# lesterphillip/SVCC23_FastSVC

Hardware: AMD Instinct MI355X
Metric: audio samples/sec (24 kHz) FastSVC generator fwd (higher is better)
Workload: dtype bf16 (bf16 MFMA products, f32 accumulate; bf16 storage); 1 GPU; cfg3: 64 x 10 s utterances per GPU, F=1500 frames, T=240000 samples, generator fastsvc.yaml (144->[192,96,48,24], x[2,4,4,5]), spk_emb on; global_batch=64, utterance_samples=240000, parallelism=utterance-parallel x1

## Files before the change

svcc23_fastsvc_amd/csrc/fastsvc_hx.hip:

```cpp
#include "fastsvc_kernels.h"

namespace fastsvc {
#ifdef FASTSVC_ACT_2B
namespace FASTSVC_ACT_NS {
#endif

#include "fastsvc_device.inc"

#include "fastsvc_hx_common.inc"

template <int MW, int NW, bool RELOAD, bool OPT_LAST = false, int NS = 3 * MW * HX_NP, int SOFF = 0, bool ADV = true>
__device__ __forceinline__ void hx_unit_direct(f32x4 (&acc)[NW][MW], const unsigned char* tile, const int (&aoff)[3],
                                               int lo_off, HxWeightStream<NS>& ws, bool do_last = true) {
    constexpr int NSTEP = 3 * NW;
    constexpr int PF = HX_NP == 1 ? (MW >= 3 ? 2 : 3) : 1;
    HxFrag a[PF + 1];
    #pragma unroll
    for (int q = 0; q < PF && q < NSTEP; ++q) a[q] = hx_read(tile, aoff[q / NW] + (q % NW) * 16 * HX_ROW, lo_off);
    #pragma unroll
    for (int s = 0; s < NSTEP; ++s) {
        const int tap = s / NW, n = s % NW;
        if (s + PF < NSTEP) {
            a[(s + PF) % (PF + 1)] = hx_read(tile, aoff[(s + PF) / NW] + ((s + PF) % NW) * 16 * HX_ROW, lo_off);
            __builtin_amdgcn_sched_barrier(0);
        }
        if (!OPT_LAST || n + 1 < NW || do_last) hx_step<MW, OPT_LAST>(acc[n], a[s % (PF + 1)], &ws.wr[SOFF + tap * MW * HX_NP]);
        if (RELOAD && n + 1 == NW) {
            #pragma unroll
            for (int q = 0; q < MW * HX_NP; ++q) ws.request(SOFF + tap * MW * HX_NP + q);
        }
        __builtin_amdgcn_sched_barrier(0);
    }
    if (RELOAD && ADV) ws.advance();
}

template <int MW, int NW>
__device__ __forceinline__ void hx_unit_direct_wl(f32x4 (&acc)[NW][MW], const unsigned char* tile, const int (&aoff)[3],
                                                  int lo_off, const unsigned char* wl, int lane) {
    constexpr int NSTEP = 3 * NW;
    HxFrag a[2];
    u32x4 w[2][MW * HX_NP];
    a[0] = hx_read(tile, aoff[0], lo_off);
    #pragma unroll
    for (int q = 0; q < MW * HX_NP; ++q) w[0][q] = *reinterpret_cast<const u32x4*>(wl + q * HX_FRAG + lane * 16);
    #pragma unroll
    for (int s = 0; s < NSTEP; ++s) {
        const int tap = s / NW, n = s % NW;
        if (s + 1 < NSTEP) {
            a[(s + 1) & 1] = hx_read(tile, aoff[(s + 1) / NW] + ((s + 1) % NW) * 16 * HX_ROW, lo_off);
            if (n + 1 == NW) {
                #pragma unroll
                for (int q = 0; q < MW * HX_NP; ++q)
                    w[(tap + 1) & 1][q] = *reinterpret_cast<const u32x4*>(wl + ((tap + 1) * MW * HX_NP + q) * HX_FRAG + lane * 16);
            }
            __builtin_amdgcn_sched_barrier(0);
        }
        hx_step<MW>(acc[n], a[s & 1], &w[tap & 1][0]);
        __builtin_amdgcn_sched_barrier(0);
    }
}

template <int MW, int NW, bool RELOAD>
__device__ __forceinline__ void hx_unit_poly(f32x4 (&acc)[3][NW][MW], const unsigned char* tile, const int (&aoff)[3],
                                             int lo_off, HxWeightStream<3 * MW * HX_NP>& ws) {
    constexpr int NSTEP = 3 * NW;
    HxFrag side[2], mid[2];
// ... 328 lines not shown
        } else {
            u32x2v a0, a1, b0, b1;
            a0.x = wa.x; a0.y = wa.y; a1.x = wa.z; a1.y = wa.w; b0.x = wb.x; b0.y = wb.y; b1.x = wb.z; b1.y = wb.w;
            __builtin_amdgcn_raw_buffer_store_b64(a0, R.y, nvs >= 4 ? off : OOB_OFF, 0, FASTSVC_ST_AUX);
            __builtin_amdgcn_raw_buffer_store_b64(a1, R.y, nvs >= 8 ? off + 8 : OOB_OFF, 0, FASTSVC_ST_AUX);
            __builtin_amdgcn_raw_buffer_store_b64(b0, R.y2, nvs >= 4 ? off : OOB_OFF, 0, FASTSVC_ST_AUX);
            __builtin_amdgcn_raw_buffer_store_b64(b1, R.y2, nvs >= 8 ? off + 8 : OOB_OFF, 0, FASTSVC_ST_AUX);
        }
    }
    __builtin_amdgcn_fence(__ATOMIC_RELEASE, "wavefront");
    __builtin_amdgcn_wave_barrier();
    __builtin_amdgcn_fence(__ATOMIC_ACQUIRE, "wavefront");
}
template <int MW, int NW, int MODE> constexpr bool hx_dec2_staged() { return MODE == MODE_DEC2 && hx_dec2_patch_bytes<MW, NW>() <= 16 * 1024; }
template <int MW, int NW, int MODE, int EPI, int S>
constexpr bool hx_poly_staged() { return MODE == MODE_POLY && (EPI == EPI_AFF || EPI == EPI_PLAIN) && hx_poly_patch_bytes<MW, NW, S>() <= 16 * 1024; }
template <int MW, int NW, int MODE> constexpr bool hx_pairs_epi() { return MODE == MODE_DIRECT && NW % 2 == 0; }
#else
template <int MW, int NW, int MODE> constexpr bool hx_pairs_epi() { return false; }
template <int MW, int NW, int MODE, int EPI, int S> constexpr bool hx_poly_staged() { return false; }
template <int MW, int NW, int S> constexpr int hx_poly_patch_bytes() { return 0; }
template <int MW, int NW, int MODE> constexpr bool hx_dec2_staged() { return false; }
template <int MW, int NW> constexpr int hx_dec2_patch_bytes() { return 0; }
#endif

template <int MW, int NW, int MODE, int EPI>
constexpr bool hx_estage() {
    return MODE == MODE_DIRECT && (EPI == EPI_AFF || EPI == EPI_RES) && (hx_pairs_epi<MW, NW, MODE>() ? MW * NW <= 12 : MW * NW <= 6);
}

template <int MW, int NW, int MODE, int EPI>
constexpr bool hx_est2() { return hx_estage<MW, NW, MODE, EPI>() && MW * NW <= 4; }

template <int MW, int NW, int MODE, int EPI, int S = 1>
constexpr int hx_min_waves() {
#ifdef FASTSVC_ACT_2B
    if (MODE == MODE_DIRECT && MW == 2 && NW == 2 && EPI == EPI_AFF && S > 1) return 4;
#endif

    return (MODE == MODE_DIRECT && MW == 2 && (EPI == EPI_PLAIN || EPI == EPI_RANK1 || EPI == EPI_RES)) ? 4 : 2;
}

template <int MW, int NW, bool PAIRS>
__device__ __forceinline__ void hx_last_reduce(const ConvParams& p, const f32x4 (&acc)[NW][MW], const float (&kw)[MW],
                                               float bias, int b, int tcol0, int lane) {
    const __amdgpu_buffer_rsrc_t yr = make_rsrc(p.last_y + (long)b * p.last_y_b, p.ldy);
    #pragma unroll
    for (int n = 0; n < NW; ++n) {
        f32x4 s = acc[n][0] * kw[0];
        #pragma unroll
        for (int m = 1; m < MW; ++m) s += acc[n][m] * kw[m];
        #pragma unroll
        for (int e = 0; e < 4; ++e) {
            float v = s[e];
            v += __builtin_bit_cast(float, __builtin_amdgcn_mov_dpp(__builtin_bit_cast(int, v), 0xB1, 0xF, 0xF, true));
            v += __builtin_bit_cast(float, __builtin_amdgcn_mov_dpp(__builtin_bit_cast(int, v), 0x4E, 0xF, 0xF, true));
            v += __builtin_bit_cast(float, __builtin_amdgcn_mov_dpp(__builtin_bit_cast(int, v), 0x141, 0xF, 0xF, true));
            v += __builtin_bit_cast(float, __builtin_amdgcn_mov_dpp(__builtin_bit_cast(int, v), 0x140, 0xF, 0xF, true));
            s[e] = v;
        }
        const int t = PAIRS ? tcol0 + (n >> 1) * 32 + (lane >> 4) * 8 + (n & 1) * 4 : tcol0 + n * 16 + (lane >> 4) * 4;
        buf_store4(yr, ((lane & 15) == 0 && t < p.T) ? t * 4 : OOB_OFF, s + bias);
    }
}

#ifndef FASTSVC_HX_W8
#define FASTSVC_HX_W8 1
#endif
constexpr bool hx_w8(int MODE, bool tailk, int S) {
    return FASTSVC_HX_W8 != 0 && HX_NP == 1 && !tailk && (MODE == MODE_DIRECT || MODE == MODE_POLY || (MODE == MODE_DEC2 && S == 2));
}

template <int MW, int NW, int WM, int WN, int MODE, int EPI, int S, bool WSTATIC, bool TAILK = false>
__global__ __launch_bounds__(512, (hx_min_waves<MW, NW, MODE, EPI, S>()))
void conv_hx_kernel(const ConvParams p0) {
    constexpr bool UPH = MODE == MODE_UPHEAD;
    constexpr bool POLY = MODE == MODE_POLY, DEC2 = MODE == MODE_DEC2, CHAIN = MODE == MODE_CHAIN || MODE == MODE_CHAIN1 || UPH;
    constexpr bool IN1 = MODE == MODE_CHAIN1;
    constexpr bool WLB = MODE == MODE_CHAIN && S == 2;
    constexpr bool XR = MODE == MODE_DIRECT && S > 1;
    constexpr int NT = 16 * NW * WN;
    constexpr int NTV = CHAIN ? NT + 16 : NT;
    constexpr int HB = CHAIN ? 4 : 0;
    constexpr int NPROD_T = 256;
    constexpr bool W8 = hx_w8(MODE, TAILK, S);
    constexpr int SPARE = W8 ? 8 : 4;
    constexpr int MAXW = NTV + (MODE == MODE_DIRECT ? (W8 ? 64 : 56) : (W8 ? 16 : 8));
    constexpr int ITEMS = (MAXW + NPROD_T - 1) / NPROD_T;
    constexpr int NWS = DEC2 ? 4 : 3;
    constexpr int NVAR = DEC2 ? 2 : 1;
    constexpr int NSLOT = NWS * MW * HX_NP;
    constexpr bool TRACKS = AMAX_TRACK && ((CHAIN && MODE != MODE_UPHEAD) || (MODE == MODE_DIRECT && (EPI == EPI_RES || EPI == EPI_RANK1)));
    extern __shared__ __attribute__((aligned(16))) unsigned char smem_raw[];

    const int tid = threadIdx.x;
    const int lane = tid & 63;
    const int wave = __builtin_amdgcn_readfirstlane(tid >> 6);
    const bool producer = wave >= 4;
    const int cw = wave & 3;
    const int wave_m = cw / WN;
    const int wave_n = cw - wave_m * WN;
    const int z = blockIdx.z;
    const int sig = z / p0.B;
    const int b = z - sig * p0.B;
    ConvParams p = p0;
    if (p0.lens) {
        const int frames = p0.lens[b];
        p.T = frames * p0.len_mul;
        p.x_T = frames * p0.xlen_mul;
    }
    const int mg = blockIdx.y * WM + wave_m;
    const bool active = !producer && mg < p.ngroups;
    const int halo = (MODE == MODE_DIRECT || CHAIN) ? p.dil : 1;
    const int halo_al = W8 ? ((halo + 7) & ~7) : ((halo + 3) & ~3);
    const int W = NTV + 2 * halo_al;
    const int nch = p.nch32;
    const int CINp = nch * HX_KC;
    const int flags = p.flags;
    const int ntx = (p.T + NT - 1) / NT;
    const int tile0 = blockIdx.x * p.tpw;
    const int ntiles = min(p.tpw, ntx - tile0);
    if (ntiles <= 0) return;
    const int nunits = ntiles * (XR ? 2 * nch : nch);
#ifdef FASTSVC_TIMELINE
    const int wg_lin = blockIdx.x + gridDim.x * (blockIdx.y + gridDim.y * blockIdx.z);
    unsigned long long* tlw = (p.tl && wg_lin < p.tl_wgs) ? p.tl + ((long)wg_lin * 8 + wave) * 64 : nullptr;
    int tli = 0;
    auto stamp = [&](int tag) {
        if (tlw && lane == 0 && tli < 62) { tlw[tli++] = ((unsigned long long)tag << 56) | (__builtin_readcyclecounter() & 0x00ffffffffffffffull); }
    };
    stamp(1);
    if (tlw && lane == 0) {
        tlw[62] = __builtin_amdgcn_s_getreg(4 | (0 << 6) | (31 << 11));
        tlw[63] = __builtin_amdgcn_s_getreg(20 | (0 << 6) | (31 << 11));
    }
#else
    auto stamp = [](int) {};
#endif

    if constexpr (hx_min_waves<MW, NW, MODE, EPI, S>() >= 4) {
        const int wg_id = blockIdx.x + gridDim.x * (blockIdx.y + gridDim.y * blockIdx.z);
        if ((wg_id >> 8) & 1) {
            for (int k = 0; k < p.stagger; ++k) __builtin_amdgcn_s_sleep(16);
        }
    }
    double* sstat = reinterpret_cast<double*>(smem_raw);
    float2* ncoef = reinterpret_cast<float2*>(smem_raw + sizeof(double) * 2 * 16 * MW * WM);
    unsigned char* tiles = reinterpret_cast<unsigned char*>(ncoef + CINp + 8);
    __shared__ unsigned s_amax, s_cnt;
    __shared__ float s_inv[HX_NP == 2 ? 2 * 16 * MW * WM : 4];
    __shared__ __attribute__((aligned(16))) float s_mid[CHAIN ? 2 * (16 * MW * WM + 32) : 4];
    float sx = 1.f;
    float sx2 = 1.f;
    float s_mid_scale = 1.f;
    const int ninv = 16 * MW * p.ngroups;
    const float* invtab = (HX_NP == 2 && p.whx_inv) ? p.whx_inv + (long)sig * p.whx_inv_sig : nullptr;
    auto operand_scales = [&]() {
#ifndef FASTSVC_EXP_NOSCALE
        if constexpr (HX_NP == 2) {
            if (p.amax_in) {
                auto bound_of = [&](int entry, int s) -> float {
                    float bd = amax_read(p.amax_in, entry);
                    #pragma unroll
                    for (int j = 0; j < 2; ++j)
                        if (p.bnd_path[j]) { const float* q = p.bnd_path[j] + (long)s * p.bnd_sig[j]; bd = bd * q[0] + q[1]; }
                    return bd;
                };
                float bound = bound_of(sig * p.amax_in_sig + b, sig);
                if (p.amax_in2 > 0) bound = fmaxf(bound, bound_of(p.amax_in2 + b, 1));
                if (flags & F_PRE_NORM) bound += sqrtf((float)p.x_T);
                if constexpr (CHAIN) {
                    if (invtab) {
                        const float* cst = invtab + (UPH ? 3 : 2) * ninv;
// ... 466 lines not shown
            #pragma unroll
            for (int c = 0; c < 8; ++c) { i1w[c][0] *= sx; i1w[c][1] *= sx; i1w[c][2] *= sx; i1b[c] *= sx; }
        }
        pcommit(0, pa, oka, tiles);
        stamp(3);
        __syncthreads();
        stamp(4);
        for (int u = 0; u < nunits; u += 2) {
            pload(u + 2, pa, oka);
            stamp(9);
            pcommit(u + 1, pb, okb, tiles + bufsz);
            stamp(5);
            ppass2(u);
            __syncthreads();
            if (CHAIN && (u % nch) == nch - 1) __syncthreads();
            stamp(6);
            pload(u + 3, pb, okb);
            stamp(9);
            pcommit(u + 2, pa, oka, tiles);
            stamp(5);
            ppass2(u + 1);
            __syncthreads();
            if (CHAIN && u + 1 < nunits && ((u + 1) % nch) == nch - 1) __syncthreads();
            stamp(6);
        }
        }
    } else {
        f32x4 acc[(POLY || DEC2 || UPH) ? 1 : NW][MW];
        f32x4 acc3[3][(POLY || UPH) ? NW : 1][MW];
        f32x4 acc2[2][DEC2 ? NW : 1][MW];
        constexpr bool XSPLIT = XR && HX_NP == 2;
        f32x4 accX[XSPLIT ? NW : 1][MW];
        float s1[MW], s2[MW];
        constexpr bool GSTAT = MODE == MODE_DIRECT && (MW * NW <= 6 || (MW == 3 && NW == 4));
        double g1[GSTAT ? MW : 1], g2[GSTAT ? MW : 1];
        #pragma unroll
        for (int m = 0; m < (GSTAT ? MW : 1); ++m) g1[m] = g2[m] = 0.0;
        HxWeightStream<NSLOT> wst;
        const int wunits = UPH ? nch + 2 * p.nch32b : CHAIN ? nch + p.nch32b : XR ? 2 * nch : nch;
        wst.init(reinterpret_cast<const unsigned char*>(p.whx) + (long)sig * p.whx_sig +
                     (long)(active ? mg : 0) * wunits * NSLOT * HX_FRAG, WLB ? nch : wunits, lane);
        int aoff[3];
        #pragma unroll
        for (int tap = 0; tap < 3; ++tap)
            aoff[tap] = hx_lds_off((halo_al - halo) + tap * halo + wave_n * (NW * 16) + (lane & 15), lane >> 4);
        int aoffX[3];
        #pragma unroll
        for (int tap = 0; tap < 3; ++tap)
            aoffX[tap] = XR ? hx_lds_off((halo_al - 1) + tap + wave_n * (NW * 16) + (lane & 15), lane >> 4) : 0;
        HxWeightStream<NSLOT> wstX_static;
        if constexpr (XR && WSTATIC)
            wstX_static.init(reinterpret_cast<const unsigned char*>(p.whx) + (long)sig * p.whx_sig +
                                 ((long)(active ? mg : 0) * wunits + 1) * NSLOT * HX_FRAG, 1, lane);
        HxWeightStream<NSLOT>& wstX = (XR && WSTATIC) ? wstX_static : wst;
        EpiRsrc R;
        {
            const long ct = (long)p.COUT * p.ldy;
            const float* nul = p.bias;
            R.y = act_rsrc(p.y ? p.y : nul, p.y ? (long)sig * p.y_sig + (long)b * p.y_b : 0, p.y ? ct : 0);
            const bool has_y2 = DEC2 || (flags & F_AFF_OUT) != 0;
            R.y2 = act_rsrc(has_y2 ? p.y2 : nul, has_y2 ? (long)sig * p.y2_sig + (long)b * p.y2_b : 0, has_y2 ? ct : 0);
            R.res = act_rsrc(p.res ? p.res : nul, p.res ? (long)sig * p.res_sig + (long)b * p.res_b : 0, p.res ? ct : 0);
            const bool has_ss = (flags & (F_STATS | F_AFF_OUT)) != 0;
            R.ss = act_rsrc(has_ss ? p.ss_out : nul, has_ss ? (long)b * p.ss_out_b : 0, has_ss ? 2 * ct : 0);
            R.r1x = make_rsrc(p.r1x ? p.r1x + (long)sig * p.r1x_sig + (long)b * p.r1x_b : nul, p.r1x ? p.ldy : 0);
        }
        float k_bias[MW], k_bias2[MW], k_r1w[MW], k_r1b[MW];
// ... 15 lines not shown
        float t_inv[MW], t_inv2[MW];
        #pragma unroll
        for (int m = 0; m < MW; ++m) {
            const int cot = (mg * MW + m) * 16 + (lane & 15);
            const bool cok = active && cot < p.COUT;
            t_inv[m] = cok ? 1.f : 0.f; t_inv2[m] = t_inv[m];
            if constexpr (HX_NP == 2) {
                if (invtab) {
                    t_inv[m] = cok ? invtab[(CHAIN ? ninv : 0) + cot] : 0.f;
                    if constexpr (DEC2) t_inv2[m] = cok ? invtab[ninv + cot] : 0.f;
                    if constexpr (UPH) t_inv2[m] = cok ? invtab[2 * ninv + cot] : 0.f;
                    if constexpr (XR) t_inv2[m] = cok ? invtab[ninv + cot] : 0.f;
                }
            }
        }
        constexpr bool LAST_OK = MODE == MODE_DIRECT && EPI == EPI_RES && WM == 1;
        float k_last[MW];
        const float b_last = (LAST_OK && p.last_w) ? __builtin_bit_cast(float, __builtin_amdgcn_readfirstlane(__builtin_bit_cast(int, p.last_b[0]))) : 0.f;
        #pragma unroll
        for (int m = 0; m < MW; ++m) {
            const int cot = (mg * MW + m) * 16 + (lane & 15);
            k_last[m] = (LAST_OK && p.last_w && active && cot < p.COUT) ? p.last_w[cot] : 0.f;
        }
        constexpr bool EST = hx_estage<MW, NW, MODE, EPI>();
        constexpr bool PAIRS = hx_pairs_epi<MW, NW, MODE>();
        constexpr int EST_WAVE_FLOATS = EST ? (PAIRS ? MW * (NW / 2) * 256 : MW * NW * EST_ITEM_FLOATS) : 0;
        const int est_ops = EPI == EPI_RES ? 1 : p.res ? 3 : 2;
        const float* Ew = reinterpret_cast<const float*>(tiles + 2 * bufsz) + cw * (est_ops * EST_WAVE_FLOATS);
        constexpr bool EST2 = hx_est2<MW, NW, MODE, EPI>() && WSTATIC && !XR;
        const int est_set = 4 * est_ops * EST_WAVE_FLOATS;
        float* Xw = const_cast<float*>(reinterpret_cast<const float*>(tiles + 2 * bufsz)) + (EST2 ? 2 : 1) * est_set +
                    cw * (16 * 36);
        (void)Xw;
        stamp(2);
        setup_shared();
        if constexpr (HX_NP == 2) {
            const float isx = 1.0f / (CHAIN ? s_mid_scale : sx);
            if (lane < 16) {
                #pragma unroll
                for (int m = 0; m < MW; ++m) {
                    const int li = (wave_m * MW + m) * 16 + lane;
                    s_inv[li] = t_inv[m] * isx;
                    if constexpr (DEC2 || UPH) s_inv[16 * MW * WM + li] = t_inv2[m] * isx;
                }
            }
        }
        float xratio[MW];
        #pragma unroll
        for (int m = 0; m < MW; ++m) {
            xratio[m] = 0.f;
            if constexpr (XR && HX_NP == 2) {
                auto ex = [](float v) { return (int)((__builtin_bit_cast(unsigned, v) >> 23) & 0xffu); };
                const int e = ex(t_inv2[m]) - ex(t_inv[m]) + ex(sx) - ex(sx2) + 127;
                if (t_inv[m] != 0.f) xratio[m] = __builtin_bit_cast(float, (unsigned)min(254, max(1, e)) << 23);
            }
        }
        __syncthreads();
        stamp(4);
        int u = 0;
        if constexpr (CHAIN) {
            f32x4 accA[NW + 1][MW];
            const int cmidp = p.nch32b * HX_KC;
            auto fwd = [&](int m) -> float {
                if constexpr (HX_NP == 2) return __builtin_bit_cast(float, (254u << 23) - __builtin_bit_cast(unsigned, K.inv(m)));
                else return 1.f;
            };
// ... 113 lines not shown
                for (int m = 0; m < MW; ++m) { s1[m] = 0.f; s2[m] = 0.f; }
                ws_epilogue_kind<MW, NW, EPI_PLAIN, false, 0, 1>(p, R, acc, s1, s2, sig, mg, tcol0, active, lane, K, Ew);
                if constexpr (TRACKS) { if (p.amax_out) amax_tile_flush(R); }
                stamp(8);
                }
            }
        } else if constexpr (XR) {
            for (int tl = 0; tl < ntiles; ++tl) {
                #pragma unroll
                for (int n = 0; n < NW; ++n)
                    #pragma unroll
                    for (int m = 0; m < MW; ++m) {
                        acc[n][m] = f32x4{0.f, 0.f, 0.f, 0.f};
                        if constexpr (XSPLIT) accX[n][m] = f32x4{0.f, 0.f, 0.f, 0.f};
                    }
                const int tcolw = (tile0 + tl) * NT + wave_n * (NW * 16);
                for (int ch = 0; ch < nch; ++ch) {
                    if constexpr (EST) {
                        if (active && ch + 1 == nch) {
#ifdef FASTSVC_ACT_2B
                            if constexpr (PAIRS) hx_epilogue8_stage<MW, NW / 2, EPI>(p, R, Ew, mg, tcolw, lane);
                            else
#endif
                            ws_epilogue_stage<MW, NW, EPI>(p, R, Ew, mg, tcolw, lane);
                        }
                    }
                    if (active) hx_unit_direct<MW, NW, !WSTATIC>(acc, tiles, aoff, lo_off, wst);
                    stamp(7);
                    __syncthreads();
                    stamp(6);
                    ++u;
                    if (active) {
                        if constexpr (XSPLIT) hx_unit_direct<MW, NW, !WSTATIC>(accX, tiles + bufsz, aoffX, lo_off, wstX);
                        else hx_unit_direct<MW, NW, !WSTATIC>(acc, tiles + bufsz, aoffX, lo_off, wstX);
                    }
                    stamp(7);
                    if (ch + 1 == nch) {
                        if constexpr (XSPLIT) {
                            #pragma unroll
                            for (int n = 0; n < NW; ++n)
                                #pragma unroll
                                for (int m = 0; m < MW; ++m) acc[n][m] += accX[n][m] * xratio[m];
                        }
                        #pragma unroll
                        for (int m = 0; m < MW; ++m) { s1[m] = 0.f; s2[m] = 0.f; }
                        if constexpr (EST) { if (active) ws_epilogue_stage_wait<NSLOT>(!WSTATIC); }
#ifdef FASTSVC_ACT_2B
                        if constexpr (PAIRS) hx_epilogue8<MW, NW / 2, EPI, EST, false, false>(p, R, acc, s1, s2, sig, mg, tcolw, active, lane, K, Ew, Xw);
                        else
#endif
                        ws_epilogue_kind<MW, NW, EPI, EST, 0, -1>(p, R, acc, s1, s2, sig, mg, tcolw, active, lane, K, Ew);
                        if (flags & F_STATS) {
                            #pragma unroll
                            for (int m = 0; m < MW; ++m) {
                                if constexpr (GSTAT) { g1[m] += (double)s1[m]; g2[m] += (double)s2[m]; }
                                else {
                                    float a1 = s1[m], a2 = s2[m];
                                    a1 = row_xsum(a1); a2 = row_xsum(a2);
                                    if (active && lane < 16) {
                                        const int slot = ((wave_m * MW + m) * 16 + lane) * 2;
                                        atomicAdd(&sstat[slot + 0], (double)a1);
                                        atomicAdd(&sstat[slot + 1], (double)a2);
                                    }
                                }
                            }
                        }
                    }
                    stamp(8);
                    __syncthreads();
                    stamp(6);
                    ++u;
                }
            }
        } else
        for (int tl = 0; tl < ntiles; ++tl) {
            auto est_stage = [&](const float* slots, int tile) {
                if constexpr (EST) {
#ifdef FASTSVC_ACT_2B
                    if constexpr (PAIRS) hx_epilogue8_stage<MW, NW / 2, EPI>(p, R, slots, mg, tile * NT + wave_n * (NW * 16), lane);
                    else
#endif
                    ws_epilogue_stage<MW, NW, EPI>(p, R, slots, mg, tile * NT + wave_n * (NW * 16), lane);
                }
            };
            #pragma unroll
            for (int n = 0; n < NW; ++n)
                #pragma unroll
                for (int m = 0; m < MW; ++m) {
                    if constexpr (POLY) { acc3[0][n][m] = acc3[1][n][m] = acc3[2][n][m] = f32x4{0.f, 0.f, 0.f, 0.f}; }
                    else if constexpr (DEC2) { acc2[0][n][m] = acc2[1][n][m] = f32x4{0.f, 0.f, 0.f, 0.f}; }
                    else acc[n][m] = f32x4{0.f, 0.f, 0.f, 0.f};
                }
            const float* EwT = EST2 ? Ew + (tl & 1) * est_set : Ew;
            for (int ch = 0; ch < nch; ++ch, ++u) {
                if constexpr (EST2) {
                    if (active && !(FASTSVC_DBG_ON(p, DBG_NO_EPILOGUE))) {
                        if (tl == 0) est_stage(Ew, tile0);
                        if (tl + 1 < ntiles) est_stage(Ew + ((tl + 1) & 1) * est_set, tile0 + tl + 1);
                    }
                } else if constexpr (EST) {
                    if (active && ch == max(nch - 2, 0) && !(FASTSVC_DBG_ON(p, DBG_NO_EPILOGUE))) est_stage(Ew, tile0 + tl);
                }
                if (active && !(FASTSVC_DBG_ON(p, DBG_NO_MFMA))) {
                    if constexpr (POLY) hx_unit_poly<MW, NW, !WSTATIC>(acc3, tiles + (u & 1) * bufsz, aoff, lo_off, wst);
                    else if constexpr (DEC2) hx_unit_dec2<MW, NW, !WSTATIC>(acc2, tiles + (u & 1) * bufsz, aoff, lo_off, raw_off, wst);
                    else hx_unit_direct<MW, NW, !WSTATIC>(acc, tiles + (u & 1) * bufsz, aoff, lo_off, wst);
                }
                stamp(7);
                if (ch + 1 == nch) {
                    #pragma unroll
                    for (int m = 0; m < MW; ++m) { s1[m] = 0.f; s2[m] = 0.f; }
                    if constexpr (EST2) {
                        if (active) {
                            constexpr int PER_OP = PAIRS ? MW * (NW / 2) : MW * NW * EST_DMA_PER_ITEM;
                            constexpr int EITEMS = PAIRS ? MW * (NW / 2) : MW * NW;
                            const int ndma = tl + 1 < ntiles ? (EPI == EPI_RES ? 1 : p.res ? 3 : 2) * PER_OP : 0;
                            int nst = 0;
                            if (tl > 0 && !(FASTSVC_DBG_ON(p, DBG_NO_EPILOGUE))) {
                                if (EPI == EPI_AFF) nst = EITEMS * (p.y ? 2 : 1);
                                else nst = (p.y ? EITEMS : 0) + ((LAST_OK && p.last_w) ? NW : 0);
                            }
                            hx_wait_vmcnt(ndma + nst);
                        }
                    } else
                    if constexpr (EST) { if (active) ws_epilogue_stage_wait<NSLOT>(!WSTATIC && !(FASTSVC_DBG_ON(p, DBG_NO_MFMA))); }
                    stamp(10);
                    if constexpr (POLY) {
#ifdef FASTSVC_ACT_2B
                        if constexpr (hx_poly_staged<MW, NW, MODE, EPI, S>()) {
                            const int tcolw = (tile0 + tl) * NT + wave_n * (NW * 16);
                            unsigned char* Pw = tiles + 2 * bufsz + cw * hx_poly_patch_bytes<MW, NW, S>();
                            HxPolyPass2<MW, NW, EPI, S, 0, hx_poly_mc<MW>()> P2;
                            if (active) {
                                P2.request(p, R, mg, tcolw, lane);
                                hx_poly_pass1<MW, NW, S>(p, acc3, mg, lane, K, Pw);
                            }
                            __syncthreads();
                            if (active) P2.run(p, R, Pw, s1, s2, mg, tcolw, lane);
                        } else
                            hx_epilogue_poly8<MW, NW, EPI, S, TAILK>(p, R, acc3, s1, s2, mg, (tile0 + tl) * NT + wave_n * (NW * 16), active, lane, K);
#else
                        ws_epilogue_poly<MW, NW, EPI, S, TAILK ? 2 : 0>(p, R, acc3, s1, s2, mg, (tile0 + tl) * NT + wave_n * (NW * 16), active, lane, K);
#endif
                    }
                    else if constexpr (DEC2)
                    {
#ifdef FASTSVC_ACT_2B
                        if constexpr (hx_dec2_staged<MW, NW, MODE>())
                            hx_epilogue_dec2_staged<MW, NW>(p, R, acc2, sig, mg, (tile0 + tl) * NT + wave_n * (NW * 16), active, lane, K,
                                                            tiles + 2 * bufsz + cw * hx_dec2_patch_bytes<MW, NW>());
                        else
#endif
                        ws_epilogue_dec2<MW, NW>(p, R, acc2, sig, mg, (tile0 + tl) * NT + wave_n * (NW * 16), active, lane, K);
                    }
                    else {
#ifdef FASTSVC_ACT_2B
                        if constexpr (PAIRS) {
                            if (!(FASTSVC_DBG_ON(p, DBG_NO_EPILOGUE)))
                                hx_epilogue8<MW, NW / 2, EPI, EST, TAILK>(p, R, acc, s1, s2, sig, mg,
                                                                   (tile0 + tl) * NT + wave_n * (NW * 16), active, lane, K, EwT, Xw);
                        } else
#endif
                        ws_epilogue_kind<MW, NW, EPI, EST, TAILK ? 2 : 0, -1>(p, R, acc, s1, s2, sig, mg,
                                                              (tile0 + tl) * NT + wave_n * (NW * 16), active, lane, K, EwT);
                        if constexpr (LAST_OK) {
                            if (p.last_w && !(FASTSVC_DBG_ON(p, DBG_NO_EPILOGUE)))
                                hx_last_reduce<MW, NW, PAIRS>(p, acc, k_last, b_last, b, (tile0 + tl) * NT + wave_n * (NW * 16), lane);
                        }
                    }
                    stamp(11);
                    if constexpr (TRACKS) { if (p.amax_out) amax_tile_flush(R); }
                    if ((flags & F_STATS) && !(FASTSVC_DBG_ON(p, DBG_NO_EPILOGUE))) {
                        #pragma unroll
                        for (int m = 0; m < MW; ++m) {
                            if constexpr (GSTAT) { g1[m] += (double)s1[m]; g2[m] += (double)s2[m]; }
                            else {
                                float a1 = s1[m], a2 = s2[m];
                                a1 = row_xsum(a1); a2 = row_xsum(a2);
                                if (active && lane < 16) {
                                    const int slot = ((wave_m * MW + m) * 16 + lane) * 2;
                                    atomicAdd(&sstat[slot + 0], (double)a1);
                                    atomicAdd(&sstat[slot + 1], (double)a2);
                                }
                            }
                        }
                    }
                }
                stamp(8);
                __syncthreads();
                stamp(6);
            }
        }
        if constexpr (TRACKS) amax_flush(p, R, &s_amax, &s_cnt, 4, sig, b, lane, blockIdx.x);
        if constexpr (GSTAT) {
            if ((flags & F_STATS) && !(FASTSVC_DBG_ON(p, DBG_NO_EPILOGUE))) {
                #pragma unroll
                for (int m = 0; m < MW; ++m) {
                    double a1 = g1[m], a2 = g2[m];
                    a1 += __shfl_xor(a1, 16); a2 += __shfl_xor(a2, 16);
                    a1 += __shfl_xor(a1, 32); a2 += __shfl_xor(a2, 32);
                    if (active && lane < 16) {
                        const int slot = ((wave_m * MW + m) * 16 + lane) * 2;
                        atomicAdd(&sstat[slot + 0], a1);
                        atomicAdd(&sstat[slot + 1], a2);
                    }
                }
            }
        }
        if (nunits & 1) __syncthreads();
    }
    if ((flags & F_STATS) && !(FASTSVC_DBG_ON(p, DBG_NO_EPILOGUE))) {
        __syncthreads();
        for (int i = tid; i < 2 * 16 * MW * WM; i += 512) {
            const int co = blockIdx.y * (WM * MW * 16) + (i >> 1);
            if (co < p.COUT) atomicAdd(&p.st_out[((long)b * p.COUT + co) * 2 + (i & 1)], sstat[i]);
        }
    }
}

constexpr size_t HX_STATIC_LDS = 4096;
template <auto KERNEL>
static hipError_t hx_launch_instance(dim3 grid, size_t smem, hipStream_t stream, const ConvParams& p) {
    if (smem + HX_STATIC_LDS > 64 * 1024) {
        static const hipError_t attr = hipFuncSetAttribute(reinterpret_cast<const void*>(KERNEL),
                                                           hipFuncAttributeMaxDynamicSharedMemorySize, 160 * 1024 - HX_STATIC_LDS);
        if (attr != hipSuccess) return attr;
    }
    hipLaunchKernelGGL(KERNEL, grid, dim3(512), smem, stream, p);
    return hipGetLastError();
}

// ... 45 lines not shown
    } else if constexpr (MODE == MODE_CHAIN) {
        if (aff || smem + HX_STATIC_LDS > 160 * 1024) return hipErrorInvalidValue;
        const int kind = p.r1x ? EPI_RANK1 : p.res ? EPI_RES : EPI_PLAIN;
        const size_t wl = (size_t)p.nch32b * 3 * MW * HX_NP * HX_FRAG;
        if constexpr (WM == 1 && MW == 3) {
            if (kind == EPI_PLAIN && p.ngroups == 1 && p.nch32b > 1 && smem + wl + HX_STATIC_LDS <= 160 * 1024)
                return hx_launch_kind<MW, NW, WM, WN, MODE_CHAIN, EPI_PLAIN, 2>(grid, smem + wl, stream, p);
        }
#define FASTSVC_HXC(k) if (kind == k) return hx_launch_kind<MW, NW, WM, WN, MODE_CHAIN, k, 1>(grid, smem, stream, p);
        FASTSVC_HXC(EPI_PLAIN) FASTSVC_HXC(EPI_RES) FASTSVC_HXC(EPI_RANK1)
#undef FASTSVC_HXC
        return hipErrorInvalidValue;
    } else if constexpr (MODE == MODE_DEC2) {
        const size_t patch = hx_dec2_staged<MW, NW, MODE_DEC2>() ? 4 * (size_t)hx_dec2_patch_bytes<MW, NW>() : 0;
        if (p.s == 1 && (p.ldx & 3) == 0) return hx_launch_kind<MW, NW, WM, WN, MODE_DEC2, EPI_PLAIN, 2>(grid, smem + patch, stream, p);
        return hx_launch_kind<MW, NW, WM, WN, MODE_DEC2, EPI_PLAIN, 1>(grid, smem + patch, stream, p);
    } else if constexpr (MODE == MODE_POLY) {
#define FASTSVC_HXP(sv) \
        if (p.s == sv) return aff ? hx_launch_kind<MW, NW, WM, WN, MODE_POLY, EPI_AFF, sv>(grid, smem + (hx_poly_staged<MW, NW, MODE_POLY, EPI_AFF, sv>() ? 4 * hx_poly_patch_bytes<MW, NW, sv>() : 0), stream, p) \
                                  : hx_launch_kind<MW, NW, WM, WN, MODE_POLY, EPI_PLAIN, sv>(grid, smem + (hx_poly_staged<MW, NW, MODE_POLY, EPI_PLAIN, sv>() ? 4 * hx_poly_patch_bytes<MW, NW, sv>() : 0), stream, p);
        FASTSVC_HXP(2) FASTSVC_HXP(4) FASTSVC_HXP(5)
#undef FASTSVC_HXP
        return hipErrorInvalidValue;
    } else {
        const int kind = aff ? EPI_AFF : p.r1x ? EPI_RANK1 : p.res ? EPI_RES : EPI_PLAIN;
        size_t est = 0;
        constexpr bool PAIRS = hx_pairs_epi<MW, NW, MODE_DIRECT>();
        if ((kind == EPI_AFF && hx_estage<MW, NW, MODE_DIRECT, EPI_AFF>()) || (kind == EPI_RES && hx_estage<MW, NW, MODE_DIRECT, EPI_RES>()))
            est = sizeof(float) * 4 * (size_t)(aff ? (p.res ? 3 : 2) : 1) * (PAIRS ? MW * (NW / 2) * 256 : MW * NW * EST_ITEM_FLOATS);
        if (MW == 2 && p.nch32 == 1 && !p.x2 &&
            ((kind == EPI_AFF && hx_est2<MW, NW, MODE_DIRECT, EPI_AFF>()) || (kind == EPI_RES && hx_est2<MW, NW, MODE_DIRECT, EPI_RES>())))
            est *= 2;
        if (PAIRS) est += sizeof(float) * 4 * 16 * 36;
        if (p.x2) {
            if (kind != EPI_AFF || p.res || p.x2_T * p.s2 != p.T || (p.lens && (((p.len_mul | p.xlen_mul) & 3) != 0)))
                return hipErrorInvalidValue;
            if (w8 && p.s2 == 2 && W / p.s2 + 5 > 128) return hipErrorInvalidValue;
            if (w8 && !conv_hx_x2_rows_ok(p)) return hipErrorInvalidValue;
#define FASTSVC_HXX(sv, stat) if (p.s2 == sv) return hx_launch_instance<&conv_hx_kernel<MW, NW, WM, WN, MODE_DIRECT, EPI_AFF, sv, stat>>(grid, smem + est, stream, p);
            if constexpr (MW * NW <= 12) {
                if constexpr (MW == 2) { if (p.nch32 == 1) { FASTSVC_HXX(5, true) } }
                else { FASTSVC_HXX(2, false) FASTSVC_HXX(4, false) }
            }
#undef FASTSVC_HXX
            return hipErrorInvalidValue;
        }
#define FASTSVC_HX(k) if (kind == k) return hx_launch_kind<MW, NW, WM, WN, MODE_DIRECT, k, 1>(grid, smem + est, stream, p);
        FASTSVC_HX(EPI_PLAIN) FASTSVC_HX(EPI_RES) FASTSVC_HX(EPI_RANK1) FASTSVC_HX(EPI_AFF)
#undef FASTSVC_HX
        return hipErrorInvalidValue;
    }
}

hipError_t launch_conv_hx(const ConvParams& p, const ConvLaunch& cfg, hipStream_t stream) {
    if (p.ntaps != 3 || (p.T & 3) || !p.whx || p.nch32 * HX_KC > 512) return hipErrorInvalidValue;
#define FASTSVC_HXS(md, mw, nw, wm, wn) \
    if (cfg.MW == mw && cfg.NW == nw && cfg.WM == wm && cfg.WN == wn) \
        return hx_launch_shape<mw, nw, wm, wn, md>(p, cfg.nsig, stream);
    if (p.mode == MODE_DIRECT) {
        if (p.dil < 1 || p.dil > 28) return hipErrorInvalidValue;
        FASTSVC_HXS(MODE_DIRECT, 2, 2, 1, 4) FASTSVC_HXS(MODE_DIRECT, 2, 3, 1, 4)
        FASTSVC_HXS(MODE_DIRECT, 3, 2, 1, 4) FASTSVC_HXS(MODE_DIRECT, 3, 3, 1, 4)
        FASTSVC_HXS(MODE_DIRECT, 3, 4, 2, 2) FASTSVC_HXS(MODE_DIRECT, 3, 6, 2, 2)
        FASTSVC_HXS(MODE_DIRECT, 3, 8, 4, 1)
    } else if (p.mode == MODE_POLY) {
        if (p.dil != 1) return hipErrorInvalidValue;
// ... 58 lines not shown
```

svcc23_fastsvc_amd/csrc/fastsvc_hx_common.inc:

```

#ifdef FASTSVC_ACT_2B
#ifdef FASTSVC_ACT_F16
typedef _Float16 hx_t;
#else
typedef __bf16 hx_t;
#endif
constexpr int HX_NP = 1;
#else
typedef _Float16 hx_t;
constexpr int HX_NP = 2;
#endif
typedef hx_t hx8 __attribute__((ext_vector_type(8)));
typedef hx_t hx2 __attribute__((ext_vector_type(2)));

__device__ __forceinline__ f32x4 hx_mfma(hx8 a, hx8 b, f32x4 c) {
#if defined(FASTSVC_ACT_2B) && !defined(FASTSVC_ACT_F16)
    return __builtin_amdgcn_mfma_f32_16x16x32_bf16(a, b, c, 0, 0, 0);
#else
    return __builtin_amdgcn_mfma_f32_16x16x32_f16(a, b, c, 0, 0, 0);
#endif
}

template <bool IN1> struct HxWin { typedef act4_t type; };
template <> struct HxWin<true> { typedef f32x4 type; };
// ... 5 lines not shown
    return ((row ^ ((row >> 2) & 1)) * HX_ROW) + ((oct ^ ((row >> 1) & 2)) << 4);
}

__device__ __forceinline__ void hx_wait_vmcnt(int n) {
    if (n >= 20) asm volatile("s_waitcnt vmcnt(20)" ::: "memory");
    else if (n >= 16) asm volatile("s_waitcnt vmcnt(16)" ::: "memory");
    else if (n >= 12) asm volatile("s_waitcnt vmcnt(12)" ::: "memory");
    else if (n >= 10) asm volatile("s_waitcnt vmcnt(10)" ::: "memory");
    else if (n >= 8) asm volatile("s_waitcnt vmcnt(8)" ::: "memory");
    else if (n >= 6) asm volatile("s_waitcnt vmcnt(6)" ::: "memory");
    else if (n >= 4) asm volatile("s_waitcnt vmcnt(4)" ::: "memory");
    else if (n >= 3) asm volatile("s_waitcnt vmcnt(3)" ::: "memory");
    else if (n >= 2) asm volatile("s_waitcnt vmcnt(2)" ::: "memory");
    else if (n >= 1) asm volatile("s_waitcnt vmcnt(1)" ::: "memory");
    else asm volatile("s_waitcnt vmcnt(0)" ::: "memory");
}

template <int NSLOT>
struct HxWeightStream {
    u32x4 wr[NSLOT];
    __amdgpu_buffer_rsrc_t rsrc;
    int voff, next, total;
    __device__ __forceinline__ void init(const unsigned char* group_base, int nunits, int lane) {
        total = nunits * NSLOT * HX_FRAG;
        rsrc = __builtin_amdgcn_make_buffer_rsrc(const_cast<unsigned char*>(group_base), 0, total, 0x00020000);
        voff = lane * 16;
        #pragma unroll
        for (int s = 0; s < NSLOT; ++s) wr[s] = __builtin_amdgcn_raw_buffer_load_b128(rsrc, voff, s * HX_FRAG, 0);
        next = NSLOT * HX_FRAG;
        if (next >= total) next = 0;
    }
    __device__ __forceinline__ void request(int s) { wr[s] = __builtin_amdgcn_raw_buffer_load_b128(rsrc, voff, next + s * HX_FRAG, 0); }
    __device__ __forceinline__ void advance() { next += NSLOT * HX_FRAG; if (next >= total) next = 0; }
};

struct HxFrag { hx8 p[HX_NP]; };

__device__ __forceinline__ HxFrag hx_read(const unsigned char* tile, int off, int lo_off) {
    HxFrag f;
    f.p[0] = *reinterpret_cast<const hx8*>(tile + off);
    if constexpr (HX_NP == 2) f.p[1] = *reinterpret_cast<const hx8*>(tile + lo_off + off);
    return f;
}

template <int PROD, bool SWAP = false>
__device__ __forceinline__ f32x4 hx_prod(const HxFrag& a, const u32x4 (&w)[HX_NP], f32x4 acc) {
    constexpr int ia = (HX_NP == 2 && PROD == 2) ? 1 : 0, iw = (HX_NP == 2 && PROD == 1) ? 1 : 0;
    if constexpr (SWAP) return hx_mfma(__builtin_bit_cast(hx8, w[iw]), a.p[ia], acc);
    else return hx_mfma(a.p[ia], __builtin_bit_cast(hx8, w[iw]), acc);
}
constexpr int HX_NPROD = HX_NP == 2 ? 3 : 1;

template <int MW, bool SWAP = false>
__device__ __forceinline__ void hx_step(f32x4 (&acc)[MW], const HxFrag& a, const u32x4* w ) {
    #pragma unroll
    for (int pr = 0; pr < HX_NPROD; ++pr)
        #pragma unroll
        for (int m = 0; m < MW; ++m) {
            u32x4 wm[HX_NP];
            #pragma unroll
            for (int q = 0; q < HX_NP; ++q) wm[q] = w[m * HX_NP + q];
            if (pr == 0) acc[m] = hx_prod<0, SWAP>(a, wm, acc[m]);
            else if (pr == 1) acc[m] = hx_prod<1, SWAP>(a, wm, acc[m]);
            else acc[m] = hx_prod<2, SWAP>(a, wm, acc[m]);
        }
}
// ... 207 lines not shown
```

Before: 1.769 billion samples/s.

## Raise occupancy for MW3xNW2 affine conv by spilling stats to LDS and deferring weight reload

For the bf16 direct-mode MW=3,NW=2 affine conv kernel, raises the launch-bounds minimum waves to 4 so more waves fit per SIMD. To cut register pressure, the double-precision stats accumulators move from registers into a per-wave LDS area. The weight-stream reload for the last channel chunk is held back and issued after the epilogue, so those registers are not live across it. The cost is extra LDS traffic and a weight-load latency that the epilogue may no longer hide, plus a possible spill risk if the register budget is still too tight.

```diff
diff --git a/svcc23_fastsvc_amd/csrc/fastsvc_hx.hip b/svcc23_fastsvc_amd/csrc/fastsvc_hx.hip
--- a/svcc23_fastsvc_amd/csrc/fastsvc_hx.hip
+++ b/svcc23_fastsvc_amd/csrc/fastsvc_hx.hip
@@ -9,9 +9,9 @@
 
 #include "fastsvc_hx_common.inc"
 
-template <int MW, int NW, bool RELOAD, bool OPT_LAST = false, int NS = 3 * MW * HX_NP, int SOFF = 0, bool ADV = true>
+template <int MW, int NW, bool RELOAD, bool OPT_LAST = false, int NS = 3 * MW * HX_NP, int SOFF = 0, bool ADV = true, bool HOLD = false>
 __device__ __forceinline__ void hx_unit_direct(f32x4 (&acc)[NW][MW], const unsigned char* tile, const int (&aoff)[3],
-                                               int lo_off, HxWeightStream<NS>& ws, bool do_last = true) {
+                                               int lo_off, HxWeightStream<NS>& ws, bool do_last = true, bool hold = false) {
     constexpr int NSTEP = 3 * NW;
     constexpr int PF = HX_NP == 1 ? (MW >= 3 ? 2 : 3) : 1;
     HxFrag a[PF + 1];
@@ -25,13 +25,13 @@
             __builtin_amdgcn_sched_barrier(0);
         }
         if (!OPT_LAST || n + 1 < NW || do_last) hx_step<MW, OPT_LAST>(acc[n], a[s % (PF + 1)], &ws.wr[SOFF + tap * MW * HX_NP]);
-        if (RELOAD && n + 1 == NW) {
+        if (RELOAD && n + 1 == NW && !(HOLD && hold)) {
             #pragma unroll
             for (int q = 0; q < MW * HX_NP; ++q) ws.request(SOFF + tap * MW * HX_NP + q);
         }
         __builtin_amdgcn_sched_barrier(0);
     }
-    if (RELOAD && ADV) ws.advance();
+    if (RELOAD && ADV && !(HOLD && hold)) ws.advance();
 }
 
 template <int MW, int NW>
@@ -426,8 +426,19 @@
 template <int MW, int NW, int MODE, int EPI>
 constexpr bool hx_est2() { return hx_estage<MW, NW, MODE, EPI>() && MW * NW <= 4; }
 
-template <int MW, int NW, int MODE, int EPI, int S = 1>
+template <int MW, int NW, int MODE, int EPI, bool TAILK = false>
+constexpr bool hx_two_cu() {
+#ifdef FASTSVC_ACT_2B
+    return MODE == MODE_DIRECT && MW == 3 && NW == 2 && EPI == EPI_AFF && !TAILK;
+#else
+    return false;
+#endif
+}
+template <int MW> constexpr int hx_gsum_bytes() { return 4 * MW * 2 * 64 * (int)sizeof(double); }
+
+template <int MW, int NW, int MODE, int EPI, int S = 1, bool TAILK = false>
 constexpr int hx_min_waves() {
+    if (hx_two_cu<MW, NW, MODE, EPI, TAILK>()) return 4;
 #ifdef FASTSVC_ACT_2B
     if (MODE == MODE_DIRECT && MW == 2 && NW == 2 && EPI == EPI_AFF && S > 1) return 4;
 #endif
@@ -466,7 +477,7 @@
 }
 
 template <int MW, int NW, int WM, int WN, int MODE, int EPI, int S, bool WSTATIC, bool TAILK = false>
-__global__ __launch_bounds__(512, (hx_min_waves<MW, NW, MODE, EPI, S>()))
+__global__ __launch_bounds__(512, (hx_min_waves<MW, NW, MODE, EPI, S, TAILK>()))
 void conv_hx_kernel(const ConvParams p0) {
     constexpr bool UPH = MODE == MODE_UPHEAD;
     constexpr bool POLY = MODE == MODE_POLY, DEC2 = MODE == MODE_DEC2, CHAIN = MODE == MODE_CHAIN || MODE == MODE_CHAIN1 || UPH;
@@ -532,7 +543,7 @@
     auto stamp = [](int) {};
 #endif
 
-    if constexpr (hx_min_waves<MW, NW, MODE, EPI, S>() >= 4) {
+    if constexpr (hx_min_waves<MW, NW, MODE, EPI, S, TAILK>() >= 4) {
         const int wg_id = blockIdx.x + gridDim.x * (blockIdx.y + gridDim.y * blockIdx.z);
         if ((wg_id >> 8) & 1) {
             for (int k = 0; k < p.stagger; ++k) __builtin_amdgcn_s_sleep(16);
@@ -1065,7 +1076,8 @@
         constexpr bool XSPLIT = XR && HX_NP == 2;
         f32x4 accX[XSPLIT ? NW : 1][MW];
         float s1[MW], s2[MW];
-        constexpr bool GSTAT = MODE == MODE_DIRECT && (MW * NW <= 6 || (MW == 3 && NW == 4));
+        constexpr bool TWO = hx_two_cu<MW, NW, MODE, EPI, TAILK>();
+        constexpr bool GSTAT = !TWO && MODE == MODE_DIRECT && (MW * NW <= 6 || (MW == 3 && NW == 4));
         double g1[GSTAT ? MW : 1], g2[GSTAT ? MW : 1];
         #pragma unroll
         for (int m = 0; m < (GSTAT ? MW : 1); ++m) g1[m] = g2[m] = 0.0;
@@ -1147,6 +1159,14 @@
         float* Xw = const_cast<float*>(reinterpret_cast<const float*>(tiles + 2 * bufsz)) + (EST2 ? 2 : 1) * est_set +
                     cw * (16 * 36);
         (void)Xw;
+        double* Gw = nullptr;
+        if constexpr (TWO) {
+            Gw = reinterpret_cast<double*>(const_cast<unsigned char*>(tiles) + 2 * bufsz + sizeof(float) * (est_set + 4 * 16 * 36)) +
+                 cw * (MW * 2 * 64) + lane;
+            #pragma unroll
+            for (int q = 0; q < MW * 2; ++q) Gw[q * 64] = 0.0;
+        }
+        (void)Gw;
         stamp(2);
         setup_shared();
         if constexpr (HX_NP == 2) {
@@ -1326,6 +1346,7 @@
                     ++u;
                     if (active) {
                         if constexpr (XSPLIT) hx_unit_direct<MW, NW, !WSTATIC>(accX, tiles + bufsz, aoffX, lo_off, wstX);
+                        else if constexpr (TWO) hx_unit_direct<MW, NW, !WSTATIC, false, NSLOT, 0, true, true>(acc, tiles + bufsz, aoffX, lo_off, wstX, true, ch + 1 == nch);
                         else hx_unit_direct<MW, NW, !WSTATIC>(acc, tiles + bufsz, aoffX, lo_off, wstX);
                     }
                     stamp(7);
@@ -1338,16 +1359,18 @@
                         }
                         #pragma unroll
                         for (int m = 0; m < MW; ++m) { s1[m] = 0.f; s2[m] = 0.f; }
-                        if constexpr (EST) { if (active) ws_epilogue_stage_wait<NSLOT>(!WSTATIC); }
+                        if constexpr (EST) { if (active) ws_epilogue_stage_wait<NSLOT>(!WSTATIC && !TWO); }
 #ifdef FASTSVC_ACT_2B
                         if constexpr (PAIRS) hx_epilogue8<MW, NW / 2, EPI, EST, false, false>(p, R, acc, s1, s2, sig, mg, tcolw, active, lane, K, Ew, Xw);
                         else
 #endif
                         ws_epilogue_kind<MW, NW, EPI, EST, 0, -1>(p, R, acc, s1, s2, sig, mg, tcolw, active, lane, K, Ew);
+                        if constexpr (TWO && !WSTATIC) { if (active) wstX.refill(); }
                         if (flags & F_STATS) {
                             #pragma unroll
                             for (int m = 0; m < MW; ++m) {
-                                if constexpr (GSTAT) { g1[m] += (double)s1[m]; g2[m] += (double)s2[m]; }
+                                if constexpr (TWO) { Gw[(2 * m) * 64] += (double)s1[m]; Gw[(2 * m + 1) * 64] += (double)s2[m]; }
+                                else if constexpr (GSTAT) { g1[m] += (double)s1[m]; g2[m] += (double)s2[m]; }
                                 else {
                                     float a1 = s1[m], a2 = s2[m];
                                     a1 = row_xsum(a1); a2 = row_xsum(a2);
@@ -1398,6 +1421,7 @@
                 if (active && !(FASTSVC_DBG_ON(p, DBG_NO_MFMA))) {
                     if constexpr (POLY) hx_unit_poly<MW, NW, !WSTATIC>(acc3, tiles + (u & 1) * bufsz, aoff, lo_off, wst);
                     else if constexpr (DEC2) hx_unit_dec2<MW, NW, !WSTATIC>(acc2, tiles + (u & 1) * bufsz, aoff, lo_off, raw_off, wst);
+                    else if constexpr (TWO) hx_unit_direct<MW, NW, !WSTATIC, false, NSLOT, 0, true, true>(acc, tiles + (u & 1) * bufsz, aoff, lo_off, wst, true, ch + 1 == nch);
                     else hx_unit_direct<MW, NW, !WSTATIC>(acc, tiles + (u & 1) * bufsz, aoff, lo_off, wst);
                 }
                 stamp(7);
@@ -1417,7 +1441,7 @@
                             hx_wait_vmcnt(ndma + nst);
                         }
                     } else
-                    if constexpr (EST) { if (active) ws_epilogue_stage_wait<NSLOT>(!WSTATIC && !(FASTSVC_DBG_ON(p, DBG_NO_MFMA))); }
+                    if constexpr (EST) { if (active) ws_epilogue_stage_wait<NSLOT>(!WSTATIC && !TWO && !(FASTSVC_DBG_ON(p, DBG_NO_MFMA))); }
                     stamp(10);
                     if constexpr (POLY) {
 #ifdef FASTSVC_ACT_2B
@@ -1462,12 +1486,16 @@
                                 hx_last_reduce<MW, NW, PAIRS>(p, acc, k_last, b_last, b, (tile0 + tl) * NT + wave_n * (NW * 16), lane);
                         }
                     }
+                    if constexpr (TWO && !WSTATIC) {
+                        if (active && !(FASTSVC_DBG_ON(p, DBG_NO_MFMA))) wst.refill();
+                    }
                     stamp(11);
                     if constexpr (TRACKS) { if (p.amax_out) amax_tile_flush(R); }
                     if ((flags & F_STATS) && !(FASTSVC_DBG_ON(p, DBG_NO_EPILOGUE))) {
                         #pragma unroll
                         for (int m = 0; m < MW; ++m) {
-                            if constexpr (GSTAT) { g1[m] += (double)s1[m]; g2[m] += (double)s2[m]; }
+                            if constexpr (TWO) { Gw[(2 * m) * 64] += (double)s1[m]; Gw[(2 * m + 1) * 64] += (double)s2[m]; }
+                            else if constexpr (GSTAT) { g1[m] += (double)s1[m]; g2[m] += (double)s2[m]; }
                             else {
                                 float a1 = s1[m], a2 = s2[m];
                                 a1 = row_xsum(a1); a2 = row_xsum(a2);
@@ -1486,11 +1514,12 @@
             }
         }
         if constexpr (TRACKS) amax_flush(p, R, &s_amax, &s_cnt, 4, sig, b, lane, blockIdx.x);
-        if constexpr (GSTAT) {
+        if constexpr (GSTAT || TWO) {
             if ((flags & F_STATS) && !(FASTSVC_DBG_ON(p, DBG_NO_EPILOGUE))) {
                 #pragma unroll
                 for (int m = 0; m < MW; ++m) {
-                    double a1 = g1[m], a2 = g2[m];
+                    double a1 = g1[GSTAT ? m : 0], a2 = g2[GSTAT ? m : 0];
+                    if constexpr (TWO) { a1 = Gw[(2 * m) * 64]; a2 = Gw[(2 * m + 1) * 64]; }
                     a1 += __shfl_xor(a1, 16); a2 += __shfl_xor(a2, 16);
                     a1 += __shfl_xor(a1, 32); a2 += __shfl_xor(a2, 32);
                     if (active && lane < 16) {
@@ -1602,6 +1631,8 @@
             ((kind == EPI_AFF && hx_est2<MW, NW, MODE_DIRECT, EPI_AFF>()) || (kind == EPI_RES && hx_est2<MW, NW, MODE_DIRECT, EPI_RES>())))
             est *= 2;
         if (PAIRS) est += sizeof(float) * 4 * 16 * 36;
+        if (kind == EPI_AFF && hx_two_cu<MW, NW, MODE_DIRECT, EPI_AFF>() && !(p.lens && (((p.len_mul | p.xlen_mul) & 3) != 0)))
+            est += hx_gsum_bytes<MW>();
         if (p.x2) {
             if (kind != EPI_AFF || p.res || p.x2_T * p.s2 != p.T || (p.lens && (((p.len_mul | p.xlen_mul) & 3) != 0)))
                 return hipErrorInvalidValue;
diff --git a/svcc23_fastsvc_amd/csrc/fastsvc_hx_common.inc b/svcc23_fastsvc_amd/csrc/fastsvc_hx_common.inc
--- a/svcc23_fastsvc_amd/csrc/fastsvc_hx_common.inc
+++ b/svcc23_fastsvc_amd/csrc/fastsvc_hx_common.inc
@@ -61,6 +61,11 @@
     }
     __device__ __forceinline__ void request(int s) { wr[s] = __builtin_amdgcn_raw_buffer_load_b128(rsrc, voff, next + s * HX_FRAG, 0); }
     __device__ __forceinline__ void advance() { next += NSLOT * HX_FRAG; if (next >= total) next = 0; }
+    __device__ __forceinline__ void refill() {
+        #pragma unroll
+        for (int s = 0; s < NSLOT; ++s) request(s);
+        advance();
+    }
 };
 
 struct HxFrag { hx8 p[HX_NP]; };
```

New measurement: 1.790 billion samples/s, median of 6. 1.01x the previous value.
